# sudo-flow/zvec

Hardware: AMD Instinct MI355X
Metric: QPS @ recall@10>=0.99, 10Mx768 fp32, batch=1024 (higher is better)
Workload: dtype f32

## Files before the change

### include/zvec_hip.h

```cpp
#ifndef ZVEC_HIP_H_
#define ZVEC_HIP_H_

#include <stddef.h>
#include <stdint.h>

#ifdef __cplusplus
extern "C" {
#endif

#define ZVEC_HIP_ABI_VERSION 1

enum {
  ZVEC_HIP_DT_FP32 = 0,
  ZVEC_HIP_DT_FP16 = 1,
  ZVEC_HIP_DT_BINARY32 = 2,
  ZVEC_HIP_DT_BINARY64 = 3
};

enum {
  ZVEC_HIP_METRIC_L2 = 0,
  ZVEC_HIP_METRIC_IP = 1,
  ZVEC_HIP_METRIC_COSINE = 2,
  ZVEC_HIP_METRIC_HAMMING = 3
};
// ... 109 lines not shown
                                   float *d_out_scores, uint32_t *d_out_counts, void *stream);
int zvec_hip_flat_set_shadow(zvec_hip_flat_t h, int enable, uint32_t preselect);
int zvec_hip_flat_shadow_info(zvec_hip_flat_t h, int *enabled, uint64_t *bytes, float *max_row_error, float *max_row_norm);
int zvec_hip_flat_shadow_width(zvec_hip_flat_t h, uint32_t topk, uint32_t *rows);
int zvec_hip_flat_shadow_certify(zvec_hip_flat_t h, zvec_hip_ctx_t ctx, const void *d_queries, uint32_t count, uint32_t topk,
                                 const uint64_t *d_exclude_bitset, uint64_t *d_out_keys, float *d_out_scores, uint32_t *d_out_counts,
                                 void *stream, uint32_t *rerun);
int zvec_hip_ivf_set_shadow(zvec_hip_ivf_t h, int enable, uint32_t preselect);
int zvec_hip_ivf_shadow_info(zvec_hip_ivf_t h, int *enabled, uint64_t *bytes, float *max_row_error, float *max_row_norm);
int zvec_hip_ivf_shadow_width(zvec_hip_ivf_t h, uint32_t topk, uint32_t *rows);
int zvec_hip_ivf_shadow_certify(zvec_hip_ivf_t h, zvec_hip_ctx_t ctx, const void *d_queries, uint32_t count, uint32_t topk,
                                uint32_t nprobe, uint32_t max_scan_count, const uint64_t *d_exclude_bitset, uint64_t *d_out_keys,
                                float *d_out_scores, uint32_t *d_out_counts, void *stream, uint32_t *rerun);
int zvec_hip_ivf_search_bf(zvec_hip_ivf_t h, zvec_hip_ctx_t ctx, const void *queries,
                           uint32_t count, uint32_t topk, float threshold,
                           const uint64_t *exclude_bitset, uint64_t *out_keys, float *out_scores,
                           uint32_t *out_counts);
int zvec_hip_ivf_keep_shard(zvec_hip_ivf_t h, uint32_t shard, uint32_t nshards);
int zvec_hip_ivf_shard_map(const uint32_t *list_sizes, uint32_t nlist, uint32_t nshards, uint32_t *owner_out,
                           uint64_t *shard_rows_out);
int zvec_hip_ivf_list_owners(zvec_hip_ivf_t h, uint32_t *owner_out);

int zvec_hip_ivf_train_dev(zvec_hip_ivf_t h, const void *d_sample, uint64_t n_sample, uint32_t nlist,
                           uint32_t kmeans_iters, uint64_t seed, void *stream);
int zvec_hip_ivf_set_centroids(zvec_hip_ivf_t h, const void *centroids, uint32_t nlist);
int zvec_hip_ivf_get_centroids(zvec_hip_ivf_t h, void *centroids, uint32_t *nlist);
int zvec_hip_ivf_label_dev(zvec_hip_ivf_t h, const void *d_rows, uint64_t n, uint32_t *d_labels, void *stream);
int zvec_hip_ivf_begin_lists(zvec_hip_ivf_t h, const uint32_t *list_sizes);
int zvec_hip_ivf_add_dev(zvec_hip_ivf_t h, const void *d_rows, uint64_t n, const uint32_t *labels,
                         const uint64_t *keys, uint64_t first_row, void *stream);
int zvec_hip_ivf_end_lists(zvec_hip_ivf_t h);
int zvec_hip_ivf_last_stats(zvec_hip_ivf_t h, zvec_hip_ctx_t ctx, uint32_t count,
                            uint32_t *scanned, uint32_t *probes);

int zvec_hip_merge_topk(zvec_hip_ctx_t ctx, const uint64_t *keys, const float *scores,
                        const uint32_t *counts, uint32_t nparts, uint32_t count, uint32_t topk,
                        uint64_t *out_keys, float *out_scores, uint32_t *out_counts);
int zvec_hip_merge_topk_dev(zvec_hip_ctx_t ctx, const uint64_t *d_keys, const float *d_scores,
                            const uint32_t *d_counts, uint32_t nparts, uint32_t count,
                            uint32_t topk, uint64_t *d_out_keys, float *d_out_scores,
                            uint32_t *d_out_counts, void *stream);

uint64_t zvec_hip_packed_bytes(uint32_t count, uint32_t topk);
int zvec_hip_merge_topk_packed_dev(zvec_hip_ctx_t ctx, const void *d_packed, uint64_t part_stride,
                                   uint32_t nparts, uint32_t count, uint32_t topk, uint64_t *d_out_keys,
                                   float *d_out_scores, uint32_t *d_out_counts, void *stream);

enum { ZVEC_HIP_SHARDS_FLAT = 0, ZVEC_HIP_SHARDS_IVF = 1 };
int zvec_hip_shards_create(uint32_t dim, int dtype, int metric, int kind, const int *devices, uint32_t ndev,
                           zvec_hip_shards_t *out);
int zvec_hip_shards_destroy(zvec_hip_shards_t h);
int zvec_hip_shards_count(zvec_hip_shards_t h, uint64_t *total, uint64_t *per_shard);
int zvec_hip_shards_flat_append(zvec_hip_shards_t h, const void *vecs, uint64_t n, const uint64_t *keys);
int zvec_hip_shards_ivf_build(zvec_hip_shards_t h, const void *vecs, uint64_t n, const uint64_t *keys, uint32_t nlist,
                              uint32_t kmeans_iters, uint32_t sample_per_list, uint64_t seed);
int zvec_hip_shards_ivf_load(zvec_hip_shards_t h, const void *centroids, uint32_t nlist, const uint64_t *list_offsets,
                             const void *vecs, const uint64_t *keys);
int zvec_hip_shards_ivf_load_segments(zvec_hip_shards_t h, const void *inverted_header, uint64_t header_bytes,
                                      const void *inverted_meta, uint64_t meta_bytes, const void *inverted_body,
                                      uint64_t body_bytes, const void *keys, uint64_t keys_bytes, const void *centroids);
int zvec_hip_shards_flat_load_features(zvec_hip_shards_t h, const void *features, uint64_t bytes, uint64_t count,
                                       int column_major, uint32_t batch_size, const uint64_t *keys);
int zvec_hip_shards_flat_search_by_ids(zvec_hip_shards_t h, const void *queries, uint32_t count, const uint64_t *ids,
                                       const uint32_t *offsets, uint32_t topk, float threshold, const uint64_t *exclude_bitset,
                                       uint64_t *out_keys, float *out_scores, uint32_t *out_counts);
int zvec_hip_shards_flat_get_vectors(zvec_hip_shards_t h, const uint64_t *positions, uint64_t n, void *out);
// ... 135 lines not shown
```

### zvec_amd/_lib.py

```python
import ctypes as C
import os

from . import build as _build

_f32p = C.c_void_p
_valp = C.c_void_p
_u64p = C.c_void_p
_u32p = C.c_void_p
_h = C.c_void_p

class DocFilterDesc(C.Structure):
    _fields_ = [("delete_bitmap", C.c_void_p), ("delete_bytes", C.c_uint64), ("delete_kind", C.c_int32),
                ("reserved_", C.c_int32), ("invert_bitmap", C.c_void_p), ("invert_bytes", C.c_uint64),
                ("forward_bits", C.c_void_p), ("forward_len", C.c_uint64)]


class Segment(C.Structure):
    _fields_ = [("id", C.c_char * 64), ("offset", C.c_uint64), ("size", C.c_uint64), ("padding", C.c_uint64),
                ("crc", C.c_uint32), ("reserved_", C.c_uint32)]


ROARING_NONE, ROARING_32, ROARING_64MAP, ROARING_FILE = 0, 1, 2, 3

DT_FP32, DT_FP16, DT_BINARY32, DT_BINARY64 = 0, 1, 2, 3
# ... 55 lines not shown
                                     C.c_uint32, C.c_uint64]),
    "zvec_hip_ivf_info": (C.c_int, [_h, C.POINTER(C.c_uint64), C.POINTER(C.c_uint32)]),
    "zvec_hip_ivf_export": (C.c_int, [_h, C.c_void_p, _u64p, _u64p]),
    "zvec_hip_ivf_get_vector": (C.c_int, [_h, C.c_uint64, C.c_void_p]),
    "zvec_hip_ivf_get_vectors": (C.c_int, [_h, _u64p, C.c_uint64, C.c_void_p]),
    "zvec_hip_ivf_search": (C.c_int, [_h, _h, C.c_void_p, C.c_uint32, C.c_uint32, C.c_float,
                                      C.c_uint32, C.c_uint32, _u64p, _u64p, _f32p, _u32p]),
    "zvec_hip_ivf_search_dev": (C.c_int, [_h, _h, C.c_void_p, C.c_uint32, C.c_uint32, C.c_float,
                                          C.c_uint32, C.c_uint32, _u64p, _u64p, _f32p, _u32p,
                                          C.c_void_p]),
    "zvec_hip_flat_set_shadow": (C.c_int, [_h, C.c_int, C.c_uint32]),
    "zvec_hip_flat_shadow_info": (C.c_int, [_h, C.POINTER(C.c_int), C.POINTER(C.c_uint64), C.POINTER(C.c_float), C.POINTER(C.c_float)]),
    "zvec_hip_flat_shadow_certify": (C.c_int, [_h, _h, C.c_void_p, C.c_uint32, C.c_uint32, _u64p, _u64p, _f32p, _u32p, C.c_void_p,
                                               C.POINTER(C.c_uint32)]),
    "zvec_hip_ivf_shadow_width": (C.c_int, [_h, C.c_uint32, C.POINTER(C.c_uint32)]),
    "zvec_hip_flat_shadow_width": (C.c_int, [_h, C.c_uint32, C.POINTER(C.c_uint32)]),
    "zvec_hip_ivf_set_shadow": (C.c_int, [_h, C.c_int, C.c_uint32]),
    "zvec_hip_ivf_shadow_info": (C.c_int, [_h, C.POINTER(C.c_int), C.POINTER(C.c_uint64), C.POINTER(C.c_float), C.POINTER(C.c_float)]),
    "zvec_hip_ivf_shadow_certify": (C.c_int, [_h, _h, C.c_void_p, C.c_uint32, C.c_uint32, C.c_uint32, C.c_uint32, _u64p, _u64p, _f32p,
                                              _u32p, C.c_void_p, C.POINTER(C.c_uint32)]),
    "zvec_hip_ivf_search_bf": (C.c_int, [_h, _h, C.c_void_p, C.c_uint32, C.c_uint32, C.c_float, _u64p,
                                         _u64p, _f32p, _u32p]),
    "zvec_hip_ivf_keep_shard": (C.c_int, [_h, C.c_uint32, C.c_uint32]),
    "zvec_hip_ivf_shard_map": (C.c_int, [_u32p, C.c_uint32, C.c_uint32, _u32p, _u64p]),
    "zvec_hip_ivf_list_owners": (C.c_int, [_h, _u32p]),
    "zvec_hip_ivf_train_dev": (C.c_int, [_h, C.c_void_p, C.c_uint64, C.c_uint32, C.c_uint32, C.c_uint64, C.c_void_p]),
    "zvec_hip_ivf_set_centroids": (C.c_int, [_h, C.c_void_p, C.c_uint32]),
    "zvec_hip_ivf_get_centroids": (C.c_int, [_h, C.c_void_p, C.POINTER(C.c_uint32)]),
    "zvec_hip_ivf_label_dev": (C.c_int, [_h, C.c_void_p, C.c_uint64, _u32p, C.c_void_p]),
    "zvec_hip_ivf_begin_lists": (C.c_int, [_h, _u32p]),
    "zvec_hip_ivf_add_dev": (C.c_int, [_h, C.c_void_p, C.c_uint64, _u32p, _u64p, C.c_uint64, C.c_void_p]),
    "zvec_hip_ivf_end_lists": (C.c_int, [_h]),
    "zvec_hip_ivf_last_stats": (C.c_int, [_h, _h, C.c_uint32, _u32p, _u32p]),
    "zvec_hip_merge_topk": (C.c_int, [_h, _u64p, _f32p, _u32p, C.c_uint32, C.c_uint32, C.c_uint32,
                                      _u64p, _f32p, _u32p]),
    "zvec_hip_merge_topk_dev": (C.c_int, [_h, _u64p, _f32p, _u32p, C.c_uint32, C.c_uint32, C.c_uint32,
                                          _u64p, _f32p, _u32p, C.c_void_p]),
    "zvec_hip_packed_bytes": (C.c_uint64, [C.c_uint32, C.c_uint32]),
    "zvec_hip_merge_topk_packed_dev": (C.c_int, [_h, C.c_void_p, C.c_uint64, C.c_uint32, C.c_uint32, C.c_uint32,
                                                 _u64p, _f32p, _u32p, C.c_void_p]),
    "zvec_hip_shards_create": (C.c_int, [C.c_uint32, C.c_int, C.c_int, C.c_int, C.POINTER(C.c_int), C.c_uint32, C.POINTER(_h)]),
    "zvec_hip_shards_destroy": (C.c_int, [_h]),
    "zvec_hip_shards_count": (C.c_int, [_h, C.POINTER(C.c_uint64), _u64p]),
    "zvec_hip_shards_flat_append": (C.c_int, [_h, C.c_void_p, C.c_uint64, _u64p]),
    "zvec_hip_shards_ivf_build": (C.c_int, [_h, C.c_void_p, C.c_uint64, _u64p, C.c_uint32, C.c_uint32, C.c_uint32, C.c_uint64]),
    "zvec_hip_shards_ivf_load": (C.c_int, [_h, C.c_void_p, C.c_uint32, _u64p, C.c_void_p, _u64p]),
    "zvec_hip_shards_ivf_load_segments": (C.c_int, [_h, C.c_void_p, C.c_uint64, C.c_void_p, C.c_uint64, C.c_void_p, C.c_uint64,
                                                    C.c_void_p, C.c_uint64, C.c_void_p]),
    "zvec_hip_shards_flat_load_features": (C.c_int, [_h, C.c_void_p, C.c_uint64, C.c_uint64, C.c_int, C.c_uint32, _u64p]),
    "zvec_hip_shards_flat_search_by_ids": (C.c_int, [_h, C.c_void_p, C.c_uint32, _u64p, _u32p, C.c_uint32, C.c_float, _u64p,
                                                     _u64p, _f32p, _u32p]),
    "zvec_hip_shards_flat_get_vectors": (C.c_int, [_h, _u64p, C.c_uint64, C.c_void_p]),
    "zvec_hip_shards_deal_coarse": (C.c_int, [_h, C.c_int]),
    "zvec_hip_shards_search": (C.c_int, [_h, C.c_void_p, C.c_uint32, C.c_uint32, C.c_float, C.c_uint32, C.c_uint32, _u64p,
                                         _u64p, _f32p, _u32p]),
    "zvec_hip_flat_build_filter": (C.c_int, [_h, _h, C.POINTER(DocFilterDesc), _u64p, C.c_int, C.c_void_p]),
    "zvec_hip_ivf_build_filter": (C.c_int, [_h, _h, C.POINTER(DocFilterDesc), _u64p, C.c_int, C.c_void_p]),
    "zvec_hip_reform_queries_dev": (C.c_int, [_h, C.c_void_p, C.c_uint32, C.c_uint32, C.c_int, C.c_int, C.c_void_p, C.c_void_p]),
    "zvec_hip_binary_encode_dev": (C.c_int, [_h, C.c_void_p, C.c_uint64, C.c_uint32, C.c_uint32, C.c_float, C.c_void_p, C.c_void_p]),
    "zvec_hip_binary_encode": (C.c_int, [_h, C.c_void_p, C.c_uint64, C.c_uint32, C.c_uint32, C.c_float, C.c_void_p]),
    "zvec_hip_flat_append_fp32": (C.c_int, [_h, C.c_void_p, C.c_uint64, C.c_uint32, C.c_uint32, C.c_float, _u64p]),
    "zvec_hip_flat_append_fp32_dev": (C.c_int, [_h, C.c_void_p, C.c_uint64, C.c_uint32, C.c_uint32, C.c_float, _u64p, C.c_void_p]),
    "zvec_hip_flat_search_fp32": (C.c_int, [_h, _h, C.c_void_p, C.c_uint32, C.c_float, C.c_uint32, C.c_uint32, C.c_float, _u64p,
                                            _u64p, _f32p, _u32p]),
    "zvec_hip_flat_search_fp32_dev": (C.c_int, [_h, _h, C.c_void_p, C.c_uint32, C.c_float, C.c_uint32, C.c_uint32, C.c_float, _u64p,
                                                _u64p, _f32p, _u32p, C.c_void_p]),
# ... 83 lines not shown
```

### zvec_amd/csrc/api_entry_ctx_flat.inc.h

```cpp

int zvec_hip_abi_version(void) { return ZVEC_HIP_ABI_VERSION; }

int zvec_hip_device_count(int *count) {
  if (!count) return ZVEC_HIP_ERR_INVALID_ARGUMENT;
  int n = 0;
  if (hipGetDeviceCount(&n) != hipSuccess) { *count = 0; return ZVEC_HIP_ERR_RUNTIME; }
  *count = n;
  return 0;
}

const char *zvec_hip_error_string(int code) {
  switch (code) {
    case ZVEC_HIP_OK: return "Success";
    case ZVEC_HIP_ERR_RUNTIME: return "Runtime error";
    case ZVEC_HIP_ERR_UNSUPPORTED: return "Unsupported";
    case ZVEC_HIP_ERR_OUT_OF_RANGE: return "Out of range";
    case ZVEC_HIP_ERR_NO_MEMORY: return "Not enough space";
    case ZVEC_HIP_ERR_NO_READY: return "No ready";
    case ZVEC_HIP_ERR_NO_EXIST: return "No exist";
    case ZVEC_HIP_ERR_MISMATCH: return "Mismatch";
    case ZVEC_HIP_ERR_INVALID_ARGUMENT: return "Invalid argument";
    case ZVEC_HIP_ERR_NO_INDEX_LOADED: return "No index loaded";
    case ZVEC_HIP_ERR_NO_TRAINED: return "No trained";
  }
  return "Unknown error";
}

int zvec_hip_set_option(const char *name, int value) {
  if (!name) return ZVEC_HIP_ERR_INVALID_ARGUMENT;
  if (strcmp(name, "wait") == 0) {
    if (value < 0 || value > 2) return ZVEC_HIP_ERR_INVALID_ARGUMENT;
    ropts().wait = value;
    return 0;
  }
  if (strcmp(name, "zerocopy") == 0) {
    if (value < 0 || value > 3) return ZVEC_HIP_ERR_INVALID_ARGUMENT;
    ropts().zerocopy = value;
    return 0;
  }
  if (strcmp(name, "assign256") == 0) { ropts().assign256 = value != 0; return 0; }
  if (strcmp(name, "scan256") == 0) {
    if (value < 0 || value > 2) return ZVEC_HIP_ERR_INVALID_ARGUMENT;
    ropts().scan256 = value;
    return 0;
  }
  if (strcmp(name, "sparse_group_rows") == 0) {
    if (value < 0 || value > 64) return ZVEC_HIP_ERR_INVALID_ARGUMENT;
    ropts().sparse_group_rows = value;
    return 0;
  }
  if (strcmp(name, "sparse_inverted_build") == 0) {
    if (value < 0 || value > 1) return ZVEC_HIP_ERR_INVALID_ARGUMENT;
    ropts().sparse_inverted_build = value;
    return 0;
  }
  return ZVEC_HIP_ERR_UNSUPPORTED;
}
int zvec_hip_get_option(const char *name, int *value) {
  if (!name || !value) return ZVEC_HIP_ERR_INVALID_ARGUMENT;
  if (strcmp(name, "wait") == 0) { *value = ropts().wait; return 0; }
  if (strcmp(name, "zerocopy") == 0) { *value = ropts().zerocopy; return 0; }
  if (strcmp(name, "assign256") == 0) { *value = ropts().assign256; return 0; }
  if (strcmp(name, "scan256") == 0) { *value = ropts().scan256; return 0; }
  if (strcmp(name, "sparse_group_rows") == 0) { *value = ropts().sparse_group_rows; return 0; }
  if (strcmp(name, "sparse_inverted_build") == 0) { *value = ropts().sparse_inverted_build; return 0; }
  return ZVEC_HIP_ERR_UNSUPPORTED;
}

int zvec_hip_host_alloc(uint64_t bytes, void **out) {
  if (!out || bytes == 0) return ZVEC_HIP_ERR_INVALID_ARGUMENT;
  void *p = nullptr;
  if (hipHostMalloc(&p, bytes, hipHostMallocPortable) != hipSuccess) { (void)hipGetLastError(); return ZVEC_HIP_ERR_NO_MEMORY; }
  *out = p;
  return 0;
}
int zvec_hip_host_free(void *p) {
  if (p) (void)hipHostFree(p);
  return 0;
}

int zvec_hip_ctx_create(int device, zvec_hip_ctx_t *out) {
  if (!out) return ZVEC_HIP_ERR_INVALID_ARGUMENT;
  return ctx_new(device, out);
}
int zvec_hip_ctx_destroy(zvec_hip_ctx_t ctx) { ctx_free(ctx); return 0; }
int zvec_hip_ctx_synchronize(zvec_hip_ctx_t ctx) {
  if (!ctx) return ZVEC_HIP_ERR_INVALID_ARGUMENT;
  ZCHK(hipSetDevice(ctx->device));
  ZCHK(hipStreamSynchronize(ctx->cur));
  return 0;
}
int zvec_hip_ctx_set_stream(zvec_hip_ctx_t ctx, void *stream) {
  if (!ctx) return ZVEC_HIP_ERR_INVALID_ARGUMENT;
  ctx->cur = stream ? reinterpret_cast<hipStream_t>(stream) : ctx->own;
  return 0;
}

int zvec_hip_gate_create(int device, zvec_hip_gate_t *out) {
// ... 585 lines not shown
```

### zvec_amd/csrc/api_entry_ivf.inc.h

```cpp

int zvec_hip_ivf_create(uint32_t dim, int dtype, int metric, int device, zvec_hip_ivf_t *out) {
  if (!out || dim == 0) return ZVEC_HIP_ERR_INVALID_ARGUMENT;
  if (dtype != ZVEC_HIP_DT_FP32 && dtype != ZVEC_HIP_DT_FP16) return ZVEC_HIP_ERR_UNSUPPORTED;
  if (metric < 0 || metric > 2) return ZVEC_HIP_ERR_UNSUPPORTED;
  if (metric == ZVEC_HIP_METRIC_COSINE && dim < (dtype == ZVEC_HIP_DT_FP16 ? 3u : 2u)) return ZVEC_HIP_ERR_INVALID_ARGUMENT;
  zvec_hip_ctx_s *c = nullptr;
  ZRET(ctx_new(device, &c));
  zvec_hip_ivf_s *h = new (std::nothrow) zvec_hip_ivf_s();
  if (!h) { ctx_free(c); return ZVEC_HIP_ERR_NO_MEMORY; }
  h->device = device; h->dtype = dtype; h->dim = dim; h->metric = metric; h->defctx = c;
  h->cent.configure(dim, metric, dtype);
  h->lists.configure(dim, metric, dtype);
  *out = h;
  return 0;
}

static void ivf_leave_coarse_space(zvec_hip_ivf_s *h) {
  if (!h->coarse_sep) return;
  h->cent.release();
  h->cent.n = 0;
  h->cent.configure(h->dim, h->metric, h->dtype);
  h->h_centroids.clear();
  h->coarse_sep = false;
  h->trained = false;
// ... 774 lines not shown
  Scoped<char> d_c;
  ZRET(d_c.alloc((size_t)nlist * rb));
  ZCHK(hipMemcpyAsync(d_c, centroids, (size_t)nlist * rb, hipMemcpyHostToDevice, s));
  ZRET(store_append_dev(h->cent, d_c, nlist, nullptr, s));
  ZCHK(hipStreamSynchronize(s));
  h->nlist = nlist;
  h->coarse_sep = true;
  h->trained = true;
  return 0;
}

int zvec_hip_ivf_search_coarse(zvec_hip_ivf_t h, zvec_hip_ctx_t ctx, const void *queries, const void *coarse_queries, uint32_t count,
                               uint32_t topk, float threshold, uint32_t nprobe, uint32_t max_scan_count,
                               const uint64_t *exclude_bitset, uint64_t *out_keys, float *out_scores, uint32_t *out_counts) {
  if (!h || !h->coarse_sep || !coarse_queries) return ZVEC_HIP_ERR_INVALID_ARGUMENT;
  return ivf_search_host_impl(h, ctx, queries, count, topk, threshold, nprobe, max_scan_count, 0, exclude_bitset, out_keys,
                              out_scores, out_counts, coarse_queries);
}

int zvec_hip_ivf_search(zvec_hip_ivf_t h, zvec_hip_ctx_t ctx, const void *queries, uint32_t count, uint32_t topk,
                        float threshold, uint32_t nprobe, uint32_t max_scan_count, const uint64_t *exclude_bitset,
                        uint64_t *out_keys, float *out_scores, uint32_t *out_counts) {
  return ivf_search_host_impl(h, ctx, queries, count, topk, threshold, nprobe, max_scan_count, 0, exclude_bitset,
                              out_keys, out_scores, out_counts);
}

int zvec_hip_ivf_search_bf(zvec_hip_ivf_t h, zvec_hip_ctx_t ctx, const void *queries, uint32_t count, uint32_t topk,
                           float threshold, const uint64_t *exclude_bitset, uint64_t *out_keys, float *out_scores,
                           uint32_t *out_counts) {
  return ivf_search_host_impl(h, ctx, queries, count, topk, threshold, 1, 0xffffffffu, 1, exclude_bitset, out_keys,
                              out_scores, out_counts);
}

int zvec_hip_ivf_last_stats(zvec_hip_ivf_t h, zvec_hip_ctx_t ctx, uint32_t count, uint32_t *scanned, uint32_t *probes) {
  if (!h) return ZVEC_HIP_ERR_INVALID_ARGUMENT;
  zvec_hip_ctx_s *c = ctx ? ctx : h->defctx;
  std::lock_guard<std::mutex> g(c->mu);
  if (!c->q_scanned || count > c->last_count) return ZVEC_HIP_ERR_NO_READY;
  ZCHK(hipSetDevice(h->device));
  ZCHK(hipStreamSynchronize(c->cur));
  if (scanned) ZCHK(hipMemcpy(scanned, c->q_scanned, (size_t)count * 4, hipMemcpyDeviceToHost));
  if (probes) ZCHK(hipMemcpy(probes, c->q_nprobe, (size_t)count * 4, hipMemcpyDeviceToHost));
  return 0;
}
```

### zvec_amd/csrc/api_ivf_core.inc.h

```cpp

namespace {

struct CoarseSplit {
  const uint32_t *given_idx = nullptr, *given_cnt = nullptr;
  uint32_t *out_idx = nullptr, *out_cnt = nullptr;
};

int ivf_search_core(zvec_hip_ivf_s *h, zvec_hip_ctx_s *ctx, const void *d_queries, uint32_t count, uint32_t topk,
                    float threshold, uint32_t nprobe, uint32_t max_scan_count, int brute_force,
                    const uint64_t *d_exclude, const SearchOut &out, hipStream_t stream, const void *d_coarse_queries = nullptr,
                    const CoarseSplit &coarse = CoarseSplit(), ShadowMode mode = ShadowMode()) {
  const bool given = coarse.given_idx != nullptr, coarse_only = coarse.out_idx != nullptr;
  if ((given || coarse_only) && brute_force) return ZVEC_HIP_ERR_INVALID_ARGUMENT;
  if (h->coarse_sep && !brute_force && !given && d_coarse_queries == nullptr) return ZVEC_HIP_ERR_INVALID_ARGUMENT;
  const int cus = device_cus(ctx);
  const uint32_t nlist = h->nlist;
  if (nprobe < 1) nprobe = 1;
  if (nprobe > nlist) nprobe = nlist;

  const uint64_t direct_rows = h->h_rows_of_largest.size() > nprobe ? std::max<uint64_t>(1, h->h_rows_of_largest[nprobe]) : ~0ull;
  const bool direct = !brute_force && !coarse_only && count <= (uint32_t)knobs().ivf_direct_q && (uint64_t)count * direct_rows <= (4u << 20) &&
                      (double)count * (double)direct_rows * (double)h->lists.row_bytes() <= 2.5e9 &&
                      merge_fits(topk) && merge_fits(nprobe);

  const bool sep = h->coarse_sep && !brute_force && !given;
  const bool raw_rows = !sep && direct && h->lists.dim_in == h->lists.dscan && (size_t)h->lists.dpad * 4 == h->lists.row_bytes() &&
                        (reinterpret_cast<uintptr_t>(d_queries) & 15u) == 0 &&
                        !(ctx->pin_in.dev && d_queries == ctx->pin_in.dev);
  const float *qrows = raw_rows ? reinterpret_cast<const float *>(d_queries) : nullptr;
  if (!raw_rows) {
    ZRET(prep_queries(ctx, sep ? h->cent : h->lists, sep ? d_coarse_queries : d_queries, count, FLT_MAX, stream));
    qrows = ctx->qpad.as<float>();
  }

  constexpr uint32_t RUN = 1024;
  uint32_t stride = 0, runs = 0, *d_off = nullptr;
  bool block_topk = false;
  PlanArgs dp{};
  if (direct) {
    stride = (uint32_t)((direct_rows + 63) / 64 * 64);
    if (stride > RUN) stride = (stride + RUN - 1) / RUN * RUN;
    runs = (stride + RUN - 1) / RUN;
    block_topk = runs > 1 && topk <= PKEYS_TOPK_MAX;
    ZRET(ctx->plan.ensure(((size_t)3 * count + 8) * sizeof(uint32_t)));
    uint32_t *pb = ctx->plan.as<uint32_t>();
    dp.coarse_idx = ctx->coarse_idx.as<uint32_t>(); dp.coarse_cnt = ctx->coarse_cnt.as<uint32_t>();
    dp.nq = count; dp.nprobe = nprobe; dp.nlist = nlist; dp.max_scan_count = max_scan_count; dp.brute_force = 0;
    dp.list_size = h->tab.d_size.p; dp.list_size_global = h->tab.d_size_global.p;
    dp.q_nprobe = pb; dp.q_scanned = pb + count;
    d_off = pb + 2 * (size_t)count;
    if (ctx->profile && ctx->nprof < PROFILE_MAX && ctx->stats.p) {
      dp.work_stats = ctx->stats.as<unsigned long long>() + 2 * (size_t)ctx->nprof;
    }
  }
// ... 126 lines not shown
    ZCHK(hipStreamSynchronize(stream));
    ctx->q_nprobe = nullptr; ctx->q_scanned = nullptr; ctx->last_count = 0;
    return 0;
  }
  ShadowTwin &tw = h->shadow;
  uint32_t kp = 0;
  if (tw.on && tw.st.base && mode.kind != ShadowMode::fp32_only && !brute_force && !(threshold < FLT_MAX) && topk <= 32 && tw.gov.allow()) {
    kp = tw.pick_kp(mode.kp, topk);
    if (kp <= topk || scan_lds_bytes(1, kp, true) > LDS_LIMIT - 1024) kp = 0;
  }
  const bool use_shadow = kp != 0;
  const uint32_t ks = use_shadow ? kp : topk;
  ctx->sh.count = 0;
  const uint32_t rows_per_group = 32;
  const uint64_t npairs = (uint64_t)count * (brute_force ? nlist : nprobe);
  size_t off = 0;
  auto take = [&](size_t words) { size_t o = off; off += (words + 3) & ~(size_t)3; return o; };
  size_t o_qnprobe = take(count), o_qscanned = take(count), o_qnslots = take(count), o_slotbegin = take(count + 1);
  size_t o_lcount = take(nlist), o_lfill = take(nlist), o_lqoff = take(nlist + 1), o_itemoff = take(nlist + 1);
  size_t o_queue = take(4);
  size_t o_ltpc = take(nlist);
  size_t o_total = take(4), o_csrq = take(npairs), o_csrslot = take(npairs);
  ZRET(ctx->plan.ensure(off * sizeof(uint32_t)));
  uint32_t *pb = ctx->plan.as<uint32_t>();
  uint32_t tpc = h->tiles_per_chunk;
  {
    const uint64_t lists_touched = std::min<uint64_t>(nlist, (uint64_t)count * (brute_force ? nlist : nprobe));
    const uint64_t est_tiles = std::max<uint64_t>(1, h->local_tiles * lists_touched / std::max<uint32_t>(nlist, 1));
    const uint64_t t = est_tiles / (4ull * (uint64_t)device_cus(ctx) * 3ull);
    const uint64_t lo = est_tiles >= 4096 ? 4 : 2;
    tpc = (uint32_t)std::min<uint64_t>(h->tiles_per_chunk, std::max<uint64_t>(lo, t));
    if (knobs().ivf_tpc) tpc = (uint32_t)knobs().ivf_tpc;
  }
  {
    ZRET(ctx->gtau.ensure((size_t)count * sizeof(uint32_t)));
    const uint32_t nzero = (uint32_t)(o_lqoff - o_lcount);
    const uint32_t nthr = std::max<uint32_t>(std::max<uint32_t>(nzero, count), std::max<uint32_t>(nlist, 4));
    hipLaunchKernelGGL(ivf_reset_kernel, dim3((nthr + 255) / 256), dim3(256), 0, stream, pb + o_lcount, nzero, pb + o_queue,
                       ctx->gtau.as<uint32_t>(), count, threshold, pb + o_ltpc, h->tab.d_tail.p, nlist, tpc);
    ZCHK(hipGetLastError());
  }
  PlanArgs p{};
  p.coarse_idx = probe_idx; p.coarse_cnt = probe_cnt;
  p.nq = count; p.nprobe = nprobe; p.nlist = nlist; p.max_scan_count = max_scan_count; p.brute_force = brute_force;
  p.list_size = h->tab.d_size.p; p.list_size_global = h->tab.d_size_global.p; p.list_order = h->tab.d_order.p;
  p.list_tpc = pb + o_ltpc;
  p.rows_per_group = rows_per_group;
  p.q_nprobe = pb + o_qnprobe; p.q_scanned = pb + o_qscanned; p.q_nslots = pb + o_qnslots; p.slot_begin = pb + o_slotbegin;
  p.list_count = pb + o_lcount; p.list_fill = pb + o_lfill; p.list_qoff = pb + o_lqoff; p.item_off = pb + o_itemoff;
  p.total_items = pb + o_total; p.csr_q = pb + o_csrq; p.csr_slot = pb + o_csrslot;
  ctx->q_nprobe = p.q_nprobe; ctx->q_scanned = p.q_scanned; ctx->last_count = count;
  ctx->last_list_count = p.list_count;
  if (ctx->profile && ctx->nprof < PROFILE_MAX && ctx->stats.p)
    p.work_stats = ctx->stats.as<unsigned long long>() + 2 * (size_t)ctx->nprof;
  hipLaunchKernelGGL(plan_wave_kernel<false>, dim3((count + 3) / 4), dim3(256), 0, stream, p);
  const bool pipelined = ctx->gate != nullptr || stream != ctx->own;
  hipLaunchKernelGGL(plan_scan_kernel, dim3(1), dim3(pipelined ? 256 : 1024), 0, stream, p);
  hipLaunchKernelGGL(plan_wave_kernel<true>, dim3((count + 3) / 4), dim3(256), 0, stream, p);
  ZCHK(hipGetLastError());

  std::vector<uint32_t> &sz = h->h_size;
  uint64_t slots_bound;
  {
    std::vector<uint32_t> chunks(nlist);
    for (uint32_t l = 0; l < nlist; ++l)
    {
      const uint32_t t = level_tpc(h->h_tail[l], tpc);
      chunks[l] = sz[l] ? (((sz[l] + TILE_N - 1) / TILE_N + t - 1) / t) : 0;
    }
    uint32_t np = brute_force ? nlist : nprobe;
    std::partial_sort(chunks.begin(), chunks.begin() + np, chunks.end(), std::greater<uint32_t>());
    uint64_t s = 0;
    for (uint32_t i = 0; i < np; ++i) s += chunks[i];
    slots_bound = s * count;
  }
  if (slots_bound == 0) slots_bound = 1;
  ZRET(ctx->part_s.ensure(slots_bound * ks * sizeof(float)));
  ZRET(ctx->part_i.ensure(slots_bound * ks * sizeof(uint32_t)));

  const StoreView &sst = use_shadow ? tw.st : h->lists;
  ScanArgs a = scan_operands(ctx, sst, d_exclude, threshold);
  if (use_shadow) {
    ZRET(shadow_prep_queries(ctx, sst, d_queries, count, stream));
    a.queries = ctx->sh.q16.as<float>(); a.qnorm = ctx->sh.qn16.as<float>();
  }
  a.k = ks; a.mode = 1; a.nq = count; a.n = h->lists.n; a.ndense = h->count_local; a.tiles_per_chunk = tpc; a.list_tpc = pb + o_ltpc;
  a.total_items = p.total_items; a.queue = pb + o_queue; a.list_order = h->tab.d_order.p; a.item_off = p.item_off; a.list_tile0 = h->tab.d_tile0.p; a.list_size = h->tab.d_size.p;
  a.list_dense0 = h->tab.d_dense0.p; a.list_qoff = p.list_qoff; a.csr_q = p.csr_q; a.csr_slot = p.csr_slot; a.nlist = nlist;
  a.part_s = ctx->part_s.as<float>(); a.part_i = ctx->part_i.as<uint32_t>();
  gate_enter(ctx, stream);
  int pi = prof_begin(ctx, stream, (double)count * sst.dscan * sst.elem + (double)count * ks * 12.0, 0, 1);
  if (pi >= 0) ctx->prof_dscan[pi] = sst.dscan | (sst.f16 ? 0x80000000u : 0u);
  const int lrc = launch_scan_ng(ng, a, sst.f16, 0x7fffffffu, cus, stream);
  prof_end(ctx, stream, pi);
  gate_leave(ctx, stream);
  ZRET(lrc);

  if (use_shadow) {
    SearchOut pre;
    ZRET(shadow_lists(ctx, count, kp, &pre));
    ZRET(launch_merge(merge_slot_ranges(a.part_s, a.part_i, p.slot_begin, kp, a.gtau, kp, threshold, h->lists.keys, pre), count,
                      merge_threads(count), stream));
    return shadow_rescore_select(ctx, h->lists, tw, count, kp, topk, out, stream);
  }
  uint32_t *ridx = out.idx;
  if (h->metric == ZVEC_HIP_METRIC_L2 && ridx == nullptr) {
    ZRET(ctx->ridx.ensure((size_t)count * topk * sizeof(uint32_t)));
    ridx = ctx->ridx.as<uint32_t>();
  }
// ... 135 lines not shown
```

### zvec_amd/csrc/api_types.inc.h

```cpp

#define ZCHK(expr)                                                                               \
  do {                                                                                           \
    hipError_t _e = (expr);                                                                      \
    if (_e != hipSuccess) {                                                                      \
      fprintf(stderr, "[zvec_hip] %s failed: %s (%s:%d)\n", #expr, hipGetErrorString(_e),        \
              __FILE__, __LINE__);                                                               \
      return (_e == hipErrorOutOfMemory) ? ZVEC_HIP_ERR_NO_MEMORY : ZVEC_HIP_ERR_RUNTIME;        \
    }                                                                                            \
  } while (0)

#define ZRET(expr)            \
  do {                        \
    int _r = (expr);          \
    if (_r != 0) return _r;   \
  } while (0)

namespace {

constexpr size_t LDS_LIMIT = 160 * 1024;
constexpr int PROFILE_MAX = 8192;

template <typename T>
struct Scoped {
  T *p = nullptr;
// ... 51 lines not shown
    const uint64_t have = std::min<uint64_t>(host.words.size(), to.cap / 8), end = hi < have ? hi + 1 : have;
    if (lo >= end) return 0;
    ZCHK(hipMemcpyAsync(to.as<uint64_t>() + lo, host.words.data() + lo, (size_t)(end - lo) * 8, hipMemcpyHostToDevice, s));
    ZCHK(hipStreamSynchronize(s));
    return 0;
  }
};

struct DevView {
  void *p = nullptr;
  template <typename T> T *as() const { return reinterpret_cast<T *>(p); }
};

struct PinnedBuf {
  void *p = nullptr;
  void *dev = nullptr;
  size_t cap = 0;
  PinnedBuf() {}
  PinnedBuf(PinnedBuf &&o) noexcept { *this = std::move(o); }
  PinnedBuf &operator=(PinnedBuf &&o) noexcept { std::swap(p, o.p); std::swap(dev, o.dev); std::swap(cap, o.cap); return *this; }
  ~PinnedBuf() { release(); }
  int ensure(size_t bytes) {
    if (bytes <= cap) return 0;
    release();
    size_t want = bytes + bytes / 4 + 256;
    ZCHK(hipHostMalloc(&p, want, hipHostMallocMapped));
    if (hipHostGetDevicePointer(&dev, p, 0) != hipSuccess) { (void)hipGetLastError(); dev = nullptr; }
    cap = want;
    return 0;
  }
  void release() { if (p) (void)hipHostFree(p); p = nullptr; dev = nullptr; cap = 0; }
};

struct RuntimeOpts {
  std::atomic<int> wait{1};
  std::atomic<int> zerocopy{2};
  std::atomic<int> assign256{1};
  std::atomic<int> scan256{1};
  std::atomic<int> sparse_group_rows{32};
  std::atomic<int> sparse_inverted_build{1};
  RuntimeOpts() {
    if (const char *e = getenv("ZVEC_HIP_SCAN256")) scan256 = std::max(0, std::min(2, atoi(e)));
    if (const char *e = getenv("ZVEC_HIP_WAIT")) wait = std::max(0, std::min(2, atoi(e)));
    if (const char *e = getenv("ZVEC_HIP_ASSIGN256")) assign256 = atoi(e) != 0;
    if (const char *e = getenv("ZVEC_HIP_ZEROCOPY")) zerocopy = std::max(0, std::min(3, atoi(e)));
  }
};
inline RuntimeOpts &ropts() {
  static RuntimeOpts o;
  return o;
}

class FairSharedMutex {
 public:
  void lock() { gate_.lock(); rw_.lock(); gate_.unlock(); }
  void unlock() { rw_.unlock(); }
  void lock_shared() { gate_.lock(); rw_.lock_shared(); gate_.unlock(); }
  void unlock_shared() { rw_.unlock_shared(); }
 private:
  std::mutex gate_;
  std::shared_mutex rw_;
};

struct ShadowGovernor {
  std::atomic<uint32_t> bad{0}, pause{0}, clean{0};
  std::atomic<int> level{0}, floor_level{-8};
  uint32_t kp_auto(uint32_t topk) const {
    const int base = (int)std::max<uint32_t>(32, 3 * topk), lo = (int)std::max<uint32_t>(16, (topk * 3 / 2 + 7) / 8 * 8);
    return (uint32_t)std::min(64, std::max(lo, base + 8 * level.load(std::memory_order_relaxed)));
  }
  void report_width(uint32_t rerun, uint32_t count) {
    if (rerun == 0) {
      if (clean.fetch_add(1, std::memory_order_relaxed) + 1 >= 6) {
// ... 187 lines not shown
struct zvec_hip_ctx_s {
  int device = 0;
  zvec_hip_gate_s *gate = nullptr;
  hipStream_t own = nullptr;
  hipStream_t cur = nullptr;
  std::mutex mu;
  DevBuf gtau, ridx;
  DevBuf seed_keys, seed_scores, seed_counts, seed_idx;
  DevBuf cmp_base, cmp_norm, cmp_extra, cmp_keys, cmp_pos, cmp_cnt;
  DevBuf qpad, qnorm, part_s, part_i, coarse_keys, coarse_scores, coarse_idx, coarse_cnt;
  DevBuf plan;
  DevBuf io_q, io_ex, io_out;
  DevBuf io_cq;
  DevView io_keys, io_scores, io_counts;
  DevBuf grp_ws, grp_of, grp_out, grp_tab;
  DevBuf direct_pos, direct_keys, direct_scores, direct_idx, direct_cnt;
  ShadowScratch sh;
  DevBuf sp_plan;
  PinnedBuf sp_pin;
  hipEvent_t sp_ev = nullptr;
  DevBuf sp_ing, sp_ing_pairs;
  DevBuf benc;
  DevBuf holes_ex;
  PinnedBuf pin_in, pin_out;
  const void *io_qp = nullptr;
  bool out_mapped = false;
  PinnedBuf done_word;
  uint32_t done_epoch = 0;
  uint64_t last_wait_ns = 0;
  hipEvent_t block_ev = nullptr;
  DevBuf stats;
  uint32_t *q_scanned = nullptr, *q_nprobe = nullptr;
  uint32_t *last_list_count = nullptr;
  uint32_t last_count = 0;
  bool profile = false;
  std::vector<hipEvent_t> ev0, ev1;
  std::vector<double> host_bytes, host_flops;
  std::vector<int> launch_is_ivf;
  std::vector<uint32_t> prof_dscan;
  int nprof = 0;
  int cus = 0;
  uint32_t route = 0;
  ~zvec_hip_ctx_s() {
    (void)hipSetDevice(device);
    if (own) (void)hipStreamSynchronize(own);
    if (block_ev) (void)hipEventDestroy(block_ev);
    if (sp_ev) (void)hipEventDestroy(sp_ev);
    for (auto e : ev0) (void)hipEventDestroy(e);
    for (auto e : ev1) (void)hipEventDestroy(e);
    if (own) (void)hipStreamDestroy(own);
  }
};

struct zvec_hip_flat_s {
  int device = 0;
  int dtype = 0;
  Store st;
  ShadowTwin shadow;
  zvec_hip_ctx_s *defctx = nullptr;
  std::mutex mu;
  FairSharedMutex rw;
  hipEvent_t append_ev = nullptr;
  bool append_pending = false;
  bool append_dirty = false;
  hipStream_t append_stream = nullptr;
  std::mutex ev_mu;
// ... 161 lines not shown
```

### zvec_amd/csrc/zvk_plan.hip.h

```cpp
#pragma once
#include "zvk_common.hip.h"

namespace zvk {

struct PlanArgs {
  const uint32_t *coarse_idx;
  const uint32_t *coarse_cnt;
  uint32_t nq, nprobe, nlist;
  uint32_t max_scan_count;
  int brute_force;
  const uint32_t *list_size;
  const uint32_t *list_size_global;
  const uint32_t *list_order;
  const uint32_t *list_tpc;
  uint32_t rows_per_group;
  uint32_t *q_nprobe;
  uint32_t *q_scanned;
  uint32_t *q_nslots;
  uint32_t *slot_begin;
  uint32_t *list_count;
  uint32_t *list_fill;
  uint32_t *list_qoff;
  uint32_t *item_off;
  uint32_t *total_items;
// ... 185 lines not shown
  block_scan([&](uint32_t i) { return p.q_nslots[i]; }, [&](uint32_t i, uint32_t v) { p.slot_begin[i] = v; },
             p.nq, &p.slot_begin[p.nq]);
  block_scan([&](uint32_t i) { return p.list_count[i]; }, [&](uint32_t i, uint32_t v) { p.list_qoff[i] = v; },
             p.nlist, &p.list_qoff[p.nlist]);
  block_scan(
      [&](uint32_t i) {
        const uint32_t l = p.list_order[i];
        uint32_t c = p.list_count[l];
        uint32_t groups = (c + p.rows_per_group - 1) / p.rows_per_group;
        return groups * list_chunks(p.list_size[l], p.list_tpc[l]);
      },
      [&](uint32_t i, uint32_t v) { p.item_off[i] = v; }, p.nlist, &p.item_off[p.nlist]);
  if (tid == 0) *p.total_items = p.item_off[p.nlist];
  if (p.work_stats) {
    __shared__ unsigned long long red[2][16];
    unsigned long long rows = 0, pairs = 0;
    for (uint32_t l = tid; l < p.nlist; l += NT) {
      const uint32_t c = p.list_count[l];
      if (c) { rows += p.list_size[l]; pairs += (unsigned long long)c * p.list_size[l]; }
    }
#pragma unroll
    for (int off = 32; off >= 1; off >>= 1) { rows += __shfl_xor(rows, off); pairs += __shfl_xor(pairs, off); }
    if (lane == 0) { red[0][wave] = rows; red[1][wave] = pairs; }
    __syncthreads();
    if (tid == 0) {
      unsigned long long r = 0, q = 0;
      for (uint32_t w = 0; w < NW; ++w) { r += red[0][w]; q += red[1][w]; }
      p.work_stats[0] = r;
      p.work_stats[1] = q;
    }
  }
}

}
```

Measured before the change: 213,200.

## Fuse IVF plan reset, wave, and scan kernels into one single-block LDS kernel

Replaces the four-kernel IVF planning sequence (reset, two plan_wave passes, plan_scan) with a single 256-thread block that keeps per-list counts and chunk counts in LDS and does the prefix scans and CSR fill in-block, when nlist is at most 8192. The host chunk-bound computation moves before the launch so max_chunks can gate the fused path. This removes launch overhead and inter-kernel gaps, but runs planning for all queries on one workgroup, so it can be slower for large batches or many probes. It also adds a debug_plan API and a runtime override for the direct-query threshold.

```diff
diff --git a/include/zvec_hip.h b/include/zvec_hip.h
--- a/include/zvec_hip.h
+++ b/include/zvec_hip.h
@@ -165,6 +165,8 @@
 int zvec_hip_ivf_end_lists(zvec_hip_ivf_t h);
 int zvec_hip_ivf_last_stats(zvec_hip_ivf_t h, zvec_hip_ctx_t ctx, uint32_t count,
                             uint32_t *scanned, uint32_t *probes);
+int zvec_hip_ivf_debug_plan(zvec_hip_ivf_t h, zvec_hip_ctx_t ctx, uint32_t which, uint32_t *out, uint64_t cap,
+                            uint64_t *words, uint32_t *route);
 
 int zvec_hip_merge_topk(zvec_hip_ctx_t ctx, const uint64_t *keys, const float *scores,
                         const uint32_t *counts, uint32_t nparts, uint32_t count, uint32_t topk,
diff --git a/zvec_amd/_lib.py b/zvec_amd/_lib.py
--- a/zvec_amd/_lib.py
+++ b/zvec_amd/_lib.py
@@ -111,6 +111,7 @@
     "zvec_hip_ivf_add_dev": (C.c_int, [_h, C.c_void_p, C.c_uint64, _u32p, _u64p, C.c_uint64, C.c_void_p]),
     "zvec_hip_ivf_end_lists": (C.c_int, [_h]),
     "zvec_hip_ivf_last_stats": (C.c_int, [_h, _h, C.c_uint32, _u32p, _u32p]),
+    "zvec_hip_ivf_debug_plan": (C.c_int, [_h, _h, C.c_uint32, _u32p, C.c_uint64, C.POINTER(C.c_uint64), _u32p]),
     "zvec_hip_merge_topk": (C.c_int, [_h, _u64p, _f32p, _u32p, C.c_uint32, C.c_uint32, C.c_uint32,
                                       _u64p, _f32p, _u32p]),
     "zvec_hip_merge_topk_dev": (C.c_int, [_h, _u64p, _f32p, _u32p, C.c_uint32, C.c_uint32, C.c_uint32,
diff --git a/zvec_amd/csrc/api_entry_ctx_flat.inc.h b/zvec_amd/csrc/api_entry_ctx_flat.inc.h
--- a/zvec_amd/csrc/api_entry_ctx_flat.inc.h
+++ b/zvec_amd/csrc/api_entry_ctx_flat.inc.h
@@ -54,6 +54,12 @@
     ropts().sparse_inverted_build = value;
     return 0;
   }
+  if (strcmp(name, "ivf_plan_fused") == 0) { ropts().ivf_plan_fused = value != 0; return 0; }
+  if (strcmp(name, "ivf_direct_q") == 0) {
+    if (value < -1) return ZVEC_HIP_ERR_INVALID_ARGUMENT;
+    ropts().ivf_direct_q = value;
+    return 0;
+  }
   return ZVEC_HIP_ERR_UNSUPPORTED;
 }
 int zvec_hip_get_option(const char *name, int *value) {
@@ -64,6 +70,8 @@
   if (strcmp(name, "scan256") == 0) { *value = ropts().scan256; return 0; }
   if (strcmp(name, "sparse_group_rows") == 0) { *value = ropts().sparse_group_rows; return 0; }
   if (strcmp(name, "sparse_inverted_build") == 0) { *value = ropts().sparse_inverted_build; return 0; }
+  if (strcmp(name, "ivf_plan_fused") == 0) { *value = ropts().ivf_plan_fused; return 0; }
+  if (strcmp(name, "ivf_direct_q") == 0) { *value = ropts().ivf_direct_q; return 0; }
   return ZVEC_HIP_ERR_UNSUPPORTED;
 }
 
diff --git a/zvec_amd/csrc/api_entry_ivf.inc.h b/zvec_amd/csrc/api_entry_ivf.inc.h
--- a/zvec_amd/csrc/api_entry_ivf.inc.h
+++ b/zvec_amd/csrc/api_entry_ivf.inc.h
@@ -830,6 +830,38 @@
                               out_scores, out_counts);
 }
 
+int zvec_hip_ivf_debug_plan(zvec_hip_ivf_t h, zvec_hip_ctx_t ctx, uint32_t which, uint32_t *out, uint64_t cap, uint64_t *words,
+                            uint32_t *route) {
+  if (!h || which >= 12) return ZVEC_HIP_ERR_INVALID_ARGUMENT;
+  zvec_hip_ctx_s *c = ctx ? ctx : h->defctx;
+  std::lock_guard<std::mutex> g(c->mu);
+  const PlanView &v = c->plan_view;
+  if (!v.route || !c->plan.p) return ZVEC_HIP_ERR_NO_READY;
+  ZCHK(hipSetDevice(h->device));
+  ZCHK(hipStreamSynchronize(c->cur));
+  const uint32_t *pb = c->plan.as<uint32_t>();
+  uint64_t n = 0;
+  switch (which) {
+    case 0: case 1: case 2: n = v.count; break;
+    case 3: n = (uint64_t)v.count + 1; break;
+    case 4: case 5: case 11: n = v.nlist; break;
+    case 6: case 7: n = (uint64_t)v.nlist + 1; break;
+    case 8: n = 1; break;
+    default: {
+      uint32_t e = 0;
+      ZCHK(hipMemcpy(&e, pb + v.off[6] + v.nlist, 4, hipMemcpyDeviceToHost));
+      n = e;
+    }
+  }
+  if (words) *words = n;
+  if (route) *route = v.route;
+  if (out) {
+    if (cap < n) return ZVEC_HIP_ERR_INVALID_ARGUMENT;
+    if (n) ZCHK(hipMemcpy(out, pb + v.off[which], (size_t)n * 4, hipMemcpyDeviceToHost));
+  }
+  return 0;
+}
+
 int zvec_hip_ivf_last_stats(zvec_hip_ivf_t h, zvec_hip_ctx_t ctx, uint32_t count, uint32_t *scanned, uint32_t *probes) {
   if (!h) return ZVEC_HIP_ERR_INVALID_ARGUMENT;
   zvec_hip_ctx_s *c = ctx ? ctx : h->defctx;
diff --git a/zvec_amd/csrc/api_ivf_core.inc.h b/zvec_amd/csrc/api_ivf_core.inc.h
--- a/zvec_amd/csrc/api_ivf_core.inc.h
+++ b/zvec_amd/csrc/api_ivf_core.inc.h
@@ -19,7 +19,9 @@
   if (nprobe > nlist) nprobe = nlist;
 
   const uint64_t direct_rows = h->h_rows_of_largest.size() > nprobe ? std::max<uint64_t>(1, h->h_rows_of_largest[nprobe]) : ~0ull;
-  const bool direct = !brute_force && !coarse_only && count <= (uint32_t)knobs().ivf_direct_q && (uint64_t)count * direct_rows <= (4u << 20) &&
+  const int direct_opt = ropts().ivf_direct_q.load(std::memory_order_relaxed);
+  const uint32_t direct_q = (uint32_t)(direct_opt >= 0 ? direct_opt : knobs().ivf_direct_q);
+  const bool direct = !brute_force && !coarse_only && count <= direct_q && (uint64_t)count * direct_rows <= (4u << 20) &&
                       (double)count * (double)direct_rows * (double)h->lists.row_bytes() <= 2.5e9 &&
                       merge_fits(topk) && merge_fits(nprobe);
 
@@ -212,14 +214,25 @@
     tpc = (uint32_t)std::min<uint64_t>(h->tiles_per_chunk, std::max<uint64_t>(lo, t));
     if (knobs().ivf_tpc) tpc = (uint32_t)knobs().ivf_tpc;
   }
+  uint64_t slots_bound;
+  uint32_t max_chunks = 0;
   {
-    ZRET(ctx->gtau.ensure((size_t)count * sizeof(uint32_t)));
-    const uint32_t nzero = (uint32_t)(o_lqoff - o_lcount);
-    const uint32_t nthr = std::max<uint32_t>(std::max<uint32_t>(nzero, count), std::max<uint32_t>(nlist, 4));
-    hipLaunchKernelGGL(ivf_reset_kernel, dim3((nthr + 255) / 256), dim3(256), 0, stream, pb + o_lcount, nzero, pb + o_queue,
-                       ctx->gtau.as<uint32_t>(), count, threshold, pb + o_ltpc, h->tab.d_tail.p, nlist, tpc);
-    ZCHK(hipGetLastError());
-  }
+    const std::vector<uint32_t> &sz = h->h_size;
+    std::vector<uint32_t> chunks(nlist);
+    for (uint32_t l = 0; l < nlist; ++l)
+    {
+      const uint32_t t = level_tpc(h->h_tail[l], tpc);
+      chunks[l] = sz[l] ? (((sz[l] + TILE_N - 1) / TILE_N + t - 1) / t) : 0;
+      max_chunks = std::max(max_chunks, chunks[l]);
+    }
+    uint32_t np = brute_force ? nlist : nprobe;
+    std::partial_sort(chunks.begin(), chunks.begin() + np, chunks.end(), std::greater<uint32_t>());
+    uint64_t s = 0;
+    for (uint32_t i = 0; i < np; ++i) s += chunks[i];
+    slots_bound = s * count;
+  }
+  if (slots_bound == 0) slots_bound = 1;
+  ZRET(ctx->gtau.ensure((size_t)count * sizeof(uint32_t)));
   PlanArgs p{};
   p.coarse_idx = probe_idx; p.coarse_cnt = probe_cnt;
   p.nq = count; p.nprobe = nprobe; p.nlist = nlist; p.max_scan_count = max_scan_count; p.brute_force = brute_force;
@@ -233,28 +246,24 @@
   ctx->last_list_count = p.list_count;
   if (ctx->profile && ctx->nprof < PROFILE_MAX && ctx->stats.p)
     p.work_stats = ctx->stats.as<unsigned long long>() + 2 * (size_t)ctx->nprof;
-  hipLaunchKernelGGL(plan_wave_kernel<false>, dim3((count + 3) / 4), dim3(256), 0, stream, p);
-  const bool pipelined = ctx->gate != nullptr || stream != ctx->own;
-  hipLaunchKernelGGL(plan_scan_kernel, dim3(1), dim3(pipelined ? 256 : 1024), 0, stream, p);
-  hipLaunchKernelGGL(plan_wave_kernel<true>, dim3((count + 3) / 4), dim3(256), 0, stream, p);
+  const bool fused = nlist <= PLAN_FUSED_MAX_NLIST && max_chunks <= 0xffffu && ropts().ivf_plan_fused.load(std::memory_order_relaxed) != 0;
+  ctx->plan_view = PlanView{fused ? 1u : 2u, count, nlist, {o_qnprobe, o_qscanned, o_qnslots, o_slotbegin, o_lcount, o_lfill, o_lqoff,
+                                                           o_itemoff, o_total, o_csrq, o_csrslot, o_ltpc}};
+  if (fused) {
+    const PlanResetArgs rs{pb + o_queue, ctx->gtau.as<uint32_t>(), threshold, pb + o_ltpc, h->tab.d_tail.p, tpc};
+    hipLaunchKernelGGL(plan_fused_kernel, dim3(1), dim3(256), plan_fused_lds_bytes(nlist), stream, p, rs);
+  } else {
+    const uint32_t nzero = (uint32_t)(o_lqoff - o_lcount);
+    const uint32_t nthr = std::max<uint32_t>(std::max<uint32_t>(nzero, count), std::max<uint32_t>(nlist, 4));
+    hipLaunchKernelGGL(ivf_reset_kernel, dim3((nthr + 255) / 256), dim3(256), 0, stream, pb + o_lcount, nzero, pb + o_queue,
+                       ctx->gtau.as<uint32_t>(), count, threshold, pb + o_ltpc, h->tab.d_tail.p, nlist, tpc);
+    hipLaunchKernelGGL(plan_wave_kernel<false>, dim3((count + 3) / 4), dim3(256), 0, stream, p);
+    const bool pipelined = ctx->gate != nullptr || stream != ctx->own;
+    hipLaunchKernelGGL(plan_scan_kernel, dim3(1), dim3(pipelined ? 256 : 1024), 0, stream, p);
+    hipLaunchKernelGGL(plan_wave_kernel<true>, dim3((count + 3) / 4), dim3(256), 0, stream, p);
+  }
   ZCHK(hipGetLastError());
 
-  std::vector<uint32_t> &sz = h->h_size;
-  uint64_t slots_bound;
-  {
-    std::vector<uint32_t> chunks(nlist);
-    for (uint32_t l = 0; l < nlist; ++l)
-    {
-      const uint32_t t = level_tpc(h->h_tail[l], tpc);
-      chunks[l] = sz[l] ? (((sz[l] + TILE_N - 1) / TILE_N + t - 1) / t) : 0;
-    }
-    uint32_t np = brute_force ? nlist : nprobe;
-    std::partial_sort(chunks.begin(), chunks.begin() + np, chunks.end(), std::greater<uint32_t>());
-    uint64_t s = 0;
-    for (uint32_t i = 0; i < np; ++i) s += chunks[i];
-    slots_bound = s * count;
-  }
-  if (slots_bound == 0) slots_bound = 1;
   ZRET(ctx->part_s.ensure(slots_bound * ks * sizeof(float)));
   ZRET(ctx->part_i.ensure(slots_bound * ks * sizeof(uint32_t)));
 
diff --git a/zvec_amd/csrc/api_types.inc.h b/zvec_amd/csrc/api_types.inc.h
--- a/zvec_amd/csrc/api_types.inc.h
+++ b/zvec_amd/csrc/api_types.inc.h
@@ -107,6 +107,12 @@
   void release() { if (p) (void)hipHostFree(p); p = nullptr; dev = nullptr; cap = 0; }
 };
 
+struct PlanView {
+  uint32_t route = 0;
+  uint32_t count = 0, nlist = 0;
+  size_t off[12] = {};
+};
+
 struct RuntimeOpts {
   std::atomic<int> wait{1};
   std::atomic<int> zerocopy{2};
@@ -114,6 +120,8 @@
   std::atomic<int> scan256{1};
   std::atomic<int> sparse_group_rows{32};
   std::atomic<int> sparse_inverted_build{1};
+  std::atomic<int> ivf_plan_fused{1};
+  std::atomic<int> ivf_direct_q{-1};
   RuntimeOpts() {
     if (const char *e = getenv("ZVEC_HIP_SCAN256")) scan256 = std::max(0, std::min(2, atoi(e)));
     if (const char *e = getenv("ZVEC_HIP_WAIT")) wait = std::max(0, std::min(2, atoi(e)));
@@ -367,6 +375,7 @@
   DevBuf stats;
   uint32_t *q_scanned = nullptr, *q_nprobe = nullptr;
   uint32_t *last_list_count = nullptr;
+  PlanView plan_view;
   uint32_t last_count = 0;
   bool profile = false;
   std::vector<hipEvent_t> ev0, ev1;
diff --git a/zvec_amd/csrc/zvk_plan.hip.h b/zvec_amd/csrc/zvk_plan.hip.h
--- a/zvec_amd/csrc/zvk_plan.hip.h
+++ b/zvec_amd/csrc/zvk_plan.hip.h
@@ -241,4 +241,167 @@
   }
 }
 
-}
+struct PlanResetArgs {
+  uint32_t *queue;
+  uint32_t *gtau;
+  float threshold;
+  uint32_t *list_tpc;
+  const uint32_t *list_tail;
+  uint32_t tpc;
+};
+
+constexpr uint32_t PLAN_FUSED_MAX_NLIST = 8192;
+__host__ __device__ inline size_t plan_fused_lds_bytes(uint32_t nlist) { return (size_t)nlist * 4 + (((size_t)nlist + 1) & ~(size_t)1) * 2; }
+
+template <class Get, class Put>
+__device__ __forceinline__ uint32_t plan_block_scan(uint32_t n, uint32_t *wtot, Get getv, Put putv) {
+  const int tid = threadIdx.x, lane = tid & 63, wave = tid >> 6;
+  const uint32_t per = (n + 255) / 256;
+  const uint32_t b = min((uint32_t)tid * per, n), e = min(b + per, n);
+  uint32_t sum = 0;
+  for (uint32_t i = b; i < e; ++i) sum += getv(i);
+  const uint32_t incl = wave_incl_scan(sum, lane);
+  __syncthreads();
+  if (lane == 63) wtot[wave] = incl;
+  __syncthreads();
+  uint32_t run = incl - sum, total = 0;
+  for (int w = 0; w < 4; ++w) { const uint32_t t = wtot[w]; if (w < wave) run += t; total += t; }
+  for (uint32_t i = b; i < e; ++i) { const uint32_t v = getv(i); putv(i, run); run += v; }
+  return total;
+}
+
+template <class F>
+__device__ __forceinline__ void plan_walk(const PlanArgs &p, uint32_t q, uint32_t np, bool vec, F f) {
+  const uint32_t *row = p.brute_force ? nullptr : p.coarse_idx + (size_t)q * p.nprobe;
+#pragma unroll 1
+  for (uint32_t r0 = 0; r0 < np; r0 += 16) {
+    uint32_t v[16];
+    if (p.brute_force) {
+#pragma unroll
+      for (int j = 0; j < 16; ++j) v[j] = r0 + j;
+    } else if (vec) {
+#pragma unroll
+      for (int j = 0; j < 4; ++j) {
+        uint4 t = make_uint4(0, 0, 0, 0);
+        if (r0 + 4 * j < np) t = *reinterpret_cast<const uint4 *>(row + r0 + 4 * j);
+        v[4 * j] = t.x; v[4 * j + 1] = t.y; v[4 * j + 2] = t.z; v[4 * j + 3] = t.w;
+      }
+    } else {
+#pragma unroll
+      for (int j = 0; j < 16; ++j) v[j] = (r0 + j < np) ? row[r0 + j] : 0u;
+    }
+#pragma unroll
+    for (int j = 0; j < 16; ++j) {
+      if (r0 + j >= np) return;
+      if (!f(v[j])) return;
+    }
+  }
+}
+
+__global__ void __launch_bounds__(256) plan_fused_kernel(const PlanArgs p, const PlanResetArgs rs) {
+  extern __shared__ uint32_t plan_lds[];
+  __shared__ uint32_t wtot[4];
+  uint32_t *cnt = plan_lds;
+  uint16_t *chs = reinterpret_cast<uint16_t *>(plan_lds + p.nlist);
+  const uint32_t tid = threadIdx.x;
+  const bool vec = !p.brute_force && (p.nprobe & 3u) == 0 && (reinterpret_cast<uintptr_t>(p.coarse_idx) & 15u) == 0;
+
+  for (uint32_t l = tid; l < p.nlist; l += 256) {
+    const uint32_t t = level_tpc(rs.list_tail[l], rs.tpc);
+    rs.list_tpc[l] = t;
+    const uint32_t szl = p.list_size[l];
+    chs[l] = (uint16_t)(szl ? list_chunks(szl, t) : 0u);
+    cnt[l] = p.list_size_global[l];
+  }
+  for (uint32_t q = tid; q < p.nq; q += 256) rs.gtau[q] = fkey(rs.threshold);
+  if (tid < 4) rs.queue[tid] = 0;
+  __syncthreads();
+
+#pragma unroll 1
+  for (uint32_t q = tid; q < p.nq; q += 256) {
+    const uint32_t np = p.brute_force ? p.nlist : min(p.coarse_cnt[q], p.nprobe);
+    uint32_t before = 0, probes = 0;
+    plan_walk(p, q, np, vec, [&](uint32_t l) {
+      if (!p.brute_force && before >= p.max_scan_count) return false;
+      before += cnt[l];
+      ++probes;
+      return true;
+    });
+    p.q_nprobe[q] = probes;
+    p.q_scanned[q] = before;
+  }
+  __syncthreads();
+  for (uint32_t l = tid; l < p.nlist; l += 256) cnt[l] = 0;
+  __syncthreads();
+
+#pragma unroll 1
+  for (uint32_t q = tid; q < p.nq; q += 256) {
+    uint32_t slots = 0;
+    plan_walk(p, q, p.q_nprobe[q], vec, [&](uint32_t l) {
+      const uint32_t c = chs[l];
+      if (c) { atomicAdd(&cnt[l], 1u); slots += c; }
+      return true;
+    });
+    p.q_nslots[q] = slots;
+  }
+  __syncthreads();
+
+  {
+    const uint32_t total = plan_block_scan(p.nq, wtot, [&](uint32_t i) { return p.q_nslots[i]; },
+                                           [&](uint32_t i, uint32_t v) { p.slot_begin[i] = v; });
+    if (tid == 0) p.slot_begin[p.nq] = total;
+  }
+  {
+    const uint32_t total = plan_block_scan(
+        p.nlist, wtot,
+        [&](uint32_t i) {
+          const uint32_t l = p.list_order[i];
+          return ((cnt[l] + p.rows_per_group - 1) / p.rows_per_group) * (uint32_t)chs[l];
+        },
+        [&](uint32_t i, uint32_t v) { p.item_off[i] = v; });
+    if (tid == 0) { p.item_off[p.nlist] = total; *p.total_items = total; }
+  }
+  if (p.work_stats) {
+    __shared__ unsigned long long red[2][4];
+    unsigned long long rows = 0, pairs = 0;
+    for (uint32_t l = tid; l < p.nlist; l += 256) {
+      const uint32_t c = cnt[l];
+      if (c) { rows += p.list_size[l]; pairs += (unsigned long long)c * p.list_size[l]; }
+    }
+#pragma unroll
+    for (int off = 32; off >= 1; off >>= 1) { rows += __shfl_xor(rows, off); pairs += __shfl_xor(pairs, off); }
+    if ((tid & 63) == 0) { red[0][tid >> 6] = rows; red[1][tid >> 6] = pairs; }
+    __syncthreads();
+    if (tid == 0) {
+      p.work_stats[0] = red[0][0] + red[0][1] + red[0][2] + red[0][3];
+      p.work_stats[1] = red[1][0] + red[1][1] + red[1][2] + red[1][3];
+    }
+  }
+  {
+    const uint32_t total = plan_block_scan(p.nlist, wtot, [&](uint32_t i) { return cnt[i]; },
+                                           [&](uint32_t i, uint32_t v) {
+                                             p.list_count[i] = p.list_fill[i] = cnt[i];
+                                             p.list_qoff[i] = v;
+                                             cnt[i] = v;
+                                           });
+    if (tid == 0) p.list_qoff[p.nlist] = total;
+  }
+  __syncthreads();
+
+#pragma unroll 1
+  for (uint32_t q = tid; q < p.nq; q += 256) {
+    uint32_t slot = p.slot_begin[q];
+    plan_walk(p, q, p.q_nprobe[q], vec, [&](uint32_t l) {
+      const uint32_t c = chs[l];
+      if (c) {
+        const uint32_t e = atomicAdd(&cnt[l], 1u);
+        p.csr_q[e] = q;
+        p.csr_slot[e] = slot;
+        slot += c;
+      }
+      return true;
+    });
+  }
+}
+
+}
```

After: 212,500. About the same (-0.3%).
